# cesar-rocha/niwqg

Measured on NVIDIA B200. Metric: fp64 grid-point-steps/sec (coupled NIW-QG), higher is better.
Workload: dtype f64

## Files before the change

### niwqg_b200/csrc/kernels_fused.cuh

```cuda
#pragma once
#include "fft_split.cuh"
#include "kernels_family.cuh"

template <int N> struct FusedGeom {
    static constexpr int R = 16, M = N / R, Nh = N / 2;
    static constexpr int NB = Nh / 64;
    static constexpr int UNITS = (M / 2) * NB;
    static constexpr size_t XSMEM = (size_t)R * 256 * sizeof(cd);
};

struct FusedThread {
    int fam;
    int n;
    int side;
    int col;
    int ptid;
    int kzero;
};

template <int N>
__host__ __device__ __forceinline__ void fused_thread(int unit, int tid, const cd* __restrict__ twc, FusedThread& t) {
    using G = FusedGeom<N>;
    const int kk = unit / G::NB;
    int b = unit % G::NB, k;
    bool self;
    if (kk == 0) { self = true; if (b < G::NB / 2) k = 0; else { k = G::M / 2; b -= G::NB / 2; } }
    else { self = false; k = kk; }
    const int half = tid >> 7, wq = (tid >> 5) & 3, lane = tid & 31;
    t.side = lane >> 4;
    const int n0 = 64 * b + 16 * wq + (lane & 15);
    if (half == 0) { t.fam = k; t.n = n0; }
    else {
        t.fam = (G::M - k) % G::M;
        t.n = (n0 == 0) ? (self ? G::Nh / 2 : 0) : G::Nh - n0;
    }
    if (n0 != 0) t.ptid = tid ^ 128 ^ 16;
    else if (!self) t.ptid = tid ^ 128;
    else t.ptid = half ? (tid ^ 16) : tid;
    t.kzero = (t.fam == 0);
    t.col = t.n + t.side * G::Nh;
}
__host__ __device__ __forceinline__ int fused_qp(const FusedThread& t, int q) { return t.kzero ? ((16 - q) & 15) : 15 - q; }

__device__ __forceinline__ cd shfl16(cd v) {
    return make_double2(__shfl_xor_sync(0xffffffffu, v.x, 16), __shfl_xor_sync(0xffffffffu, v.y, 16));
}

template <int N>
__device__ __forceinline__ void fused_combine(const cd* __restrict__ T, const cd* __restrict__ twc, const FusedThread& t, cd (&u)[16]) {
    constexpr int M = N / 16;
    cd v[16];
    const cd wx = __ldg(&twc[t.n]), wy = __ldg(&twc[t.fam]);
#pragma unroll
    for (int r = 0; r < 16; ++r) v[r] = __ldg(&T[(size_t)(r * M + t.fam) * N + t.col]);
    if (t.side) {
#pragma unroll
        for (int r = 0; r < 16; ++r) v[r] = cmul(v[r], wx);
    }
#pragma unroll
    for (int r = 0; r < 16; ++r) {
        const cd o2 = shfl16(v[r]);
        v[r] = t.side ? csub(o2, v[r]) : cadd(v[r], o2);
    }
    fftc::apply_twiddles<16, 1>(v, wy);
    fftc::dft<16, 1>(v);
#pragma unroll
    for (int p = 0; p < 16; ++p) u[fftc::outidx<16>(p)] = v[p];
}

template <int N>
__device__ __forceinline__ void fused_produce(cd (&v)[16], const cd* __restrict__ twc, const FusedThread& t, int pro, double dk,
                                              cd* __restrict__ out) {
    constexpr int M = N / 16;
    const cd wx = __ldg(&twc[t.n]), wy = __ldg(&twc[t.fam]);
#define NIWQG_PRO_CASE(P)                                                                     \
    case P:                                                                                   \
        _Pragma("unroll") for (int r = 0; r < 16; ++r) v[r] = split_prologue<N, P>(dk, t.fam + M * r, t.col, v[r]); \
        break;
    switch (pro) {
        NIWQG_PRO_CASE(PRO_IK)
        NIWQG_PRO_CASE(PRO_IL)
        NIWQG_PRO_CASE(PRO_UV)
        default: break;
    }
#undef NIWQG_PRO_CASE
#pragma unroll
    for (int r = 0; r < 16; ++r) v[r].y = -v[r].y;
#pragma unroll
    for (int r = 0; r < 16; ++r) {
        const cd o2 = shfl16(v[r]);
        v[r] = t.side ? cmul(csub(o2, v[r]), wx) : cadd(v[r], o2);
    }
    fftc::dft<16, 1>(v);
    cd u[16];
#pragma unroll
    for (int p = 0; p < 16; ++p) u[fftc::outidx<16>(p)] = v[p];
    fftc::apply_twiddles<16, 1>(u, wy);
#pragma unroll
    for (int q = 0; q < 16; ++q) out[(size_t)(q * M + t.fam) * N + t.col] = u[q];
}

struct FStageArgs {
    StageArgs s;
    const cd* T;
    cd* out[3];
    int nout;
    const cd* twc;
    double dk;
};

struct EqIn { cd y0, cur, F0, Fab, y1, c0, c1, c2, c3; double fl; };

template <int ST, bool PHI>
__device__ __forceinline__ void eq_load(EqIn& in, const cd* __restrict__ y0, const cd* y, const cd* __restrict__ y1,
                                        const cd* __restrict__ F0, const cd* Fab, const TableSet& t,
                                        const double* __restrict__ filtr, size_t i) {
    in.y0 = __ldg(&y0[i]);
    if (PHI && ST >= 2) in.cur = (ST == 2) ? __ldg(&y1[i]) : y[i];
    if (ST >= 3) { in.F0 = __ldg(&F0[i]); in.Fab = (ST == 4) ? __ldg(&Fab[i]) : Fab[i]; }
    if (ST == 3) in.y1 = __ldg(&y1[i]);
    if (ST <= 3) { in.c0 = __ldg(&t.E2[i]); in.c1 = __ldg(&t.Q[i]); }
    else { in.c0 = __ldg(&t.E[i]); in.c1 = __ldg(&t.f0[i]); in.c2 = __ldg(&t.fab[i]); in.c3 = __ldg(&t.fc[i]); }
    in.fl = __ldg(&filtr[i]);
}
template <int ST> struct FusedDepth { static constexpr int Q = ST <= 2 ? 4 : 3, PHI = ST <= 2 ? 4 : (ST == 3 ? 3 : 2), INV = 6; };
template <int ST>
__device__ __forceinline__ cd eq_update(const EqIn& in, cd y0, cd Fn, cd& F0, cd& Fab) {
    cd r;
    if (ST == 1 || ST == 2) {
        r = cadd(cmul(in.c0, y0), cmul(Fn, in.c1));
        if (ST == 1) F0 = Fn; else Fab = Fn;
    } else if (ST == 3) {
        F0 = in.F0;
        const cd c = make_double2(2.0 * Fn.x - F0.x, 2.0 * Fn.y - F0.y);
        r = cadd(cmul(in.c0, in.y1), cmul(c, in.c1));
        Fab = cadd(in.Fab, Fn);
    } else {
        const cd ab2 = make_double2(2.0 * in.Fab.x, 2.0 * in.Fab.y);
        r = cadd(cadd(cadd(cmul(in.c0, y0), cmul(in.F0, in.c1)), cmul(ab2, in.c2)), cmul(Fn, in.c3));
    }
    return make_double2(r.x * in.fl, r.y * in.fl);
}

template <int N, int ST>
__global__ void __launch_bounds__(256, 2) k_fstage_q(FStageArgs a) {
    using G = FusedGeom<N>;
    constexpr int M = G::M;
    extern __shared__ __align__(16) unsigned char fused_smem[];
    cd* xs = reinterpret_cast<cd*>(fused_smem);
    const int tid = threadIdx.x;
    for (int unit = blockIdx.x; unit < G::UNITS; unit += gridDim.x) {
        FusedThread t;
        fused_thread<N>(unit, tid, a.twc, t);
        {
            cd u[16];
            fused_combine<N>(a.T, a.twc, t, u);
#pragma unroll
            for (int q = 0; q < 16; ++q) xs[q * 256 + tid] = u[q];
        }
        __syncthreads();
        const double k1 = a.dk * (double)sidx(t.col, N);
        const size_t i0 = (size_t)t.fam * N + t.col;
        constexpr int D = FusedDepth<ST>::Q;
        EqIn in[D];
        const int ub = unit % G::NB;
        const bool nyq = (ub == 0) || (unit < G::NB && ub == G::NB / 2);
        if (a.s.hsym && !t.kzero && !nyq) {
            const int colp = (N - t.col) & (N - 1);
#pragma unroll
            for (int p = 0; p < D - 1; ++p) eq_load<ST, false>(in[p], a.s.y0q, a.s.yq, a.s.y1q, a.s.F0q, a.s.Fabq, a.s.tq, a.s.filtr, i0 + (size_t)(2 * p) * M * N);
#pragma unroll
            for (int qq = 0; qq < 8; ++qq) {
                const int q = 2 * qq;
                const int ky = t.fam + M * q;
                const size_t i1 = i0 + (size_t)q * M * N;
                const size_t ip = (size_t)(N - ky) * N + colp;
                if (qq + D - 1 < 8) eq_load<ST, false>(in[(qq + D - 1) % D], a.s.y0q, a.s.yq, a.s.y1q, a.s.F0q, a.s.Fabq, a.s.tq, a.s.filtr, i1 + (size_t)(2 * (D - 1)) * M * N);
                const cd p1 = xs[q * 256 + tid], p2 = xs[(15 - q) * 256 + t.ptid];
                const double l1 = a.dk * (double)sidx(ky, N);
                const cd A = make_double2(0.5 * (p1.x + p2.x), 0.5 * (p1.y - p2.y));
                const cd B = make_double2(0.5 * (p1.y + p2.y), -0.5 * (p1.x - p2.x));
                const cd F1 = make_double2(k1 * A.y + l1 * B.y, -(k1 * A.x + l1 * B.x));
                const EqIn& e = in[qq % D];
                cd F0a, Faba;
                const cd n1 = eq_update<ST>(e, e.y0, F1, F0a, Faba);
                const cd n1c = make_double2(n1.x, -n1.y);
                a.s.yq[i1] = n1; a.s.yq[ip] = n1c;
                if (ST == 1) {
                    a.s.F0q[i1] = F0a; a.s.F0q[ip] = make_double2(F0a.x, -F0a.y);
                    if (a.s.y1q != a.s.yq) { a.s.y1q[i1] = n1; a.s.y1q[ip] = n1c; }
                }
                if (ST == 2 || ST == 3) { a.s.Fabq[i1] = Faba; a.s.Fabq[ip] = make_double2(Faba.x, -Faba.y); }
            }
            __syncthreads();
            continue;
        }
#pragma unroll
        for (int p = 0; p < D - 1; ++p) eq_load<ST, false>(in[p], a.s.y0q, a.s.yq, a.s.y1q, a.s.F0q, a.s.Fabq, a.s.tq, a.s.filtr, i0 + (size_t)p * M * N);
#pragma unroll
        for (int q = 0; q < 16; ++q) {
            const int ky = t.fam + M * q;
            const size_t i1 = i0 + (size_t)q * M * N;
            if (q + D - 1 < 16) eq_load<ST, false>(in[(q + D - 1) % D], a.s.y0q, a.s.yq, a.s.y1q, a.s.F0q, a.s.Fabq, a.s.tq, a.s.filtr, i1 + (size_t)(D - 1) * M * N);
            const cd p1 = xs[q * 256 + tid], p2 = xs[fused_qp(t, q) * 256 + t.ptid];
            const double l1 = a.dk * (double)sidx(ky, N);
            const cd A = make_double2(0.5 * (p1.x + p2.x), 0.5 * (p1.y - p2.y));
            const cd B = make_double2(0.5 * (p1.y + p2.y), -0.5 * (p1.x - p2.x));
            cd F1 = make_double2(k1 * A.y + l1 * B.y, -(k1 * A.x + l1 * B.x));
            if (ky == 0 && t.col == 0) F1 = make_double2(0.0, 0.0);
            const EqIn& e = in[q % D];
            cd F0a, Faba;
            const cd n1 = eq_update<ST>(e, e.y0, F1, F0a, Faba);
            a.s.yq[i1] = n1;
            if (ST == 1) { a.s.F0q[i1] = F0a; if (a.s.y1q != a.s.yq) a.s.y1q[i1] = n1; }
            if (ST == 2 || ST == 3) a.s.Fabq[i1] = Faba;
        }
        __syncthreads();
    }
}

template <int N, int ST>
__global__ void __launch_bounds__(256, 2) k_fstage_phi(FStageArgs a) {
    using G = FusedGeom<N>;
    constexpr int M = G::M;
    extern __shared__ __align__(16) unsigned char fused_smem[];
    cd* xs = reinterpret_cast<cd*>(fused_smem);
    const int tid = threadIdx.x;
    __shared__ double ssum[SE_COUNT][256];
#pragma unroll
    for (int k = 0; k < SE_COUNT; ++k) ssum[k][tid] = 0.0;
    const bool specb = (a.s.flags & MF_SPEC_BUDGET) != 0;
    for (int unit = blockIdx.x; unit < G::UNITS; unit += gridDim.x) {
        FusedThread t;
        fused_thread<N>(unit, tid, a.twc, t);
        {
            cd u[16];
            fused_combine<N>(a.T, a.twc, t, u);
#pragma unroll
            for (int q = 0; q < 16; ++q) xs[q * 256 + tid] = u[q];
        }
        __syncwarp();
        const double k1 = a.dk * (double)sidx(t.col, N);
        const size_t i0 = (size_t)t.fam * N + t.col;
        double s[SE_COUNT];
#pragma unroll
        for (int k = 0; k < SE_COUNT; ++k) s[k] = 0.0;
        constexpr int D = FusedDepth<ST>::PHI;
        EqIn in[D];
#pragma unroll
        for (int p = 0; p < D - 1; ++p) eq_load<ST, true>(in[p], a.s.y0p, a.s.yp, a.s.y1p, a.s.F0p, a.s.Fabp, a.s.tp, a.s.filtr, i0 + (size_t)p * M * N);
#pragma unroll
        for (int q = 0; q < 16; ++q) {
            const int ky = t.fam + M * q;
            const size_t i1 = i0 + (size_t)q * M * N;
            if (q + D - 1 < 16) eq_load<ST, true>(in[(q + D - 1) % D], a.s.y0p, a.s.yp, a.s.y1p, a.s.F0p, a.s.Fabp, a.s.tp, a.s.filtr, i1 + (size_t)(D - 1) * M * N);
            const EqIn& e = in[q % D];
            cd F1 = xs[q * 256 + tid];
            const cd cur1 = (ST == 1) ? e.y0 : e.cur;
            if (specb || (a.s.flags & MF_HAS_LAP2)) {
                const double l1 = a.dk * (double)sidx(ky, N);
                const double wv2 = k1 * k1 + l1 * l1, w4 = wv2 * wv2;
                const double m2 = cur1.x * cur1.x + cur1.y * cur1.y;
                s[SE_LAP2] += w4 * m2;
                s[SE_WV6PHI] += w4 * wv2 * m2;
                if (specb) {
                    const double zr = cur1.x * F1.x + cur1.y * F1.y, zi = cur1.y * F1.x - cur1.x * F1.y;
                    s[SE_T0R] += zr; s[SE_T0I] += zi;
                    s[SE_T1R] += wv2 * zr; s[SE_T1I] += wv2 * zi;
                    s[SE_T2R] += w4 * zr; s[SE_T2I] += w4 * zi;
                }
            }
            if ((a.s.flags & MF_FIX00) && ky == 0 && t.col == 0) { F1.x += a.s.sumsD[SD_J_R]; F1.y += a.s.sumsD[SD_J_I]; }
            cd F0a, Faba;
            const cd n1 = eq_update<ST>(e, e.y0, F1, F0a, Faba);
            a.s.yp[i1] = n1;
            if (ST == 1) { a.s.F0p[i1] = F0a; if (a.s.y1p != a.s.yp) a.s.y1p[i1] = n1; }
            if (ST == 2 || ST == 3) a.s.Fabp[i1] = Faba;
        }
#pragma unroll
        for (int k = 0; k < SE_COUNT; ++k) ssum[k][tid] += s[k];
        for (int o = 0; o < a.nout; ++o) {
            cd v[16];
#pragma unroll
            for (int r = 0; r < 16; ++r) v[r] = a.s.yp[i0 + (size_t)r * M * N];
            fused_produce<N>(v, a.twc, t, o == 0 ? PRO_NONE : o == 1 ? PRO_IK : PRO_IL, a.dk, a.out[o]);
        }
    }
    double s[SE_COUNT];
#pragma unroll
    for (int k = 0; k < SE_COUNT; ++k) s[k] = ssum[k][tid];
    block_reduce_store<SE_COUNT>(s, a.s.partials);
}

struct FInvertArgs {
    InvertArgs i;
    const cd* T;
    cd *out_uv, *out_qs;
    const cd* twc;
    double dk;
};

struct InvIn { cd q1, q2; double fl, flp; };

template <int N, bool HASW>
__global__ void __launch_bounds__(256, 2) k_finvert(FInvertArgs a) {
    using G = FusedGeom<N>;
    constexpr int M = G::M;
    extern __shared__ __align__(16) unsigned char fused_smem[];
    cd* xs = reinterpret_cast<cd*>(fused_smem);
    const int tid = threadIdx.x;
    __shared__ double ssum[SI_COUNT][256];
#pragma unroll
    for (int k = 0; k < SI_COUNT; ++k) ssum[k][tid] = 0.0;
    for (int unit = blockIdx.x; unit < G::UNITS; unit += gridDim.x) {
        FusedThread t;
        fused_thread<N>(unit, tid, a.twc, t);
        if (HASW) {
            cd u[16];
            fused_combine<N>(a.T, a.twc, t, u);
#pragma unroll
            for (int q = 0; q < 16; ++q) xs[q * 256 + tid] = u[q];
            __syncthreads();
        }
        cd u[16];
        double s[SI_COUNT] = {0.0, 0.0, 0.0};
        const double k1 = a.dk * (double)sidx(t.col, N);
        const int colp = (N - t.col) & (N - 1);
        const size_t i0 = (size_t)t.fam * N + t.col;
        auto load = [&](InvIn& in, int q) {
            const int ky = t.fam + M * q, kyp = (N - ky) & (N - 1);
            in.q1 = __ldg(&a.i.qh[i0 + (size_t)q * M * N]);
            in.q2 = __ldg(&a.i.qh[(size_t)kyp * N + colp]);
            if (HASW) {
                in.fl = __ldg(&a.i.filtr[i0 + (size_t)q * M * N]);
                in.flp = a.i.filtr_sym ? in.fl : __ldg(&a.i.filtr[(size_t)kyp * N + colp]);
            }
        };
        constexpr int D = FusedDepth<1>::INV;
        InvIn in[D];
#pragma unroll
        for (int p = 0; p < D - 1; ++p) load(in[p], p);
#pragma unroll
        for (int q = 0; q < 16; ++q) {
            const int ky = t.fam + M * q;
            const size_t i1 = i0 + (size_t)q * M * N;
            if (q + D - 1 < 16) load(in[(q + D - 1) % D], q + D - 1);
            const InvIn& e = in[q % D];
            const double l1 = a.dk * (double)sidx(ky, N);
            const double wv2 = __dadd_rn(__dmul_rn(k1, k1), __dmul_rn(l1, l1));
            const double wv2i = (wv2 != 0.0) ? 1.0 / wv2 : 0.0;
            const cd Hq = make_double2(0.5 * (e.q1.x + e.q2.x), 0.5 * (e.q1.y - e.q2.y));
            cd qw = make_double2(0.0, 0.0), qwr = qw;
            if (HASW) {
                const cd W1 = xs[q * 256 + tid], W2 = xs[fused_qp(t, q) * 256 + t.ptid];
                const cd A = make_double2(0.5 * (W1.x + W2.x), 0.5 * (W1.y - W2.y));
                cd Jc = make_double2(a.i.inv_jscale * 0.5 * (W1.y + W2.y), a.i.inv_jscale * -0.5 * (W1.x - W2.x));
                if (ky == 0 && t.col == 0) Jc = make_double2(0.0, 0.0);
                const double bx = 0.5 * (0.5 * (-wv2 * A.x) + Jc.x) / a.i.f, by = 0.5 * (0.5 * (-wv2 * A.y) + Jc.y) / a.i.f;
                const double fs = 0.5 * (e.fl + e.flp);
                qw.x = bx * fs; qw.y = by * fs;
                qwr.x = bx * e.fl; qwr.y = by * e.fl;
            }
            const cd ph1 = make_double2(wv2i * qw.x - wv2i * Hq.x, wv2i * qw.y - wv2i * Hq.y);
            {
                const double r = Hq.x * ph1.x + Hq.y * ph1.y;
                s[SI_QLAP2PSI] += wv2 * wv2 * r;
                s[SI_PLAPQ] += -wv2 * r;
                s[SI_PQ] += r;
            }
            a.i.ph[i1] = ph1;
            if (a.i.qwh) a.i.qwh[i1] = qwr;
            u[q] = make_double2(Hq.x - qw.y, Hq.y + qw.x);
        }
        if (HASW) __syncthreads();
#pragma unroll
        for (int k = 0; k < SI_COUNT; ++k) ssum[k][tid] += s[k];
        fused_produce<N>(u, a.twc, t, PRO_NONE, a.dk, a.out_qs);
#pragma unroll
        for (int r = 0; r < 16; ++r) u[r] = a.i.ph[i0 + (size_t)r * M * N];
        fused_produce<N>(u, a.twc, t, PRO_UV, a.dk, a.out_uv);
    }
    double s[SI_COUNT];
#pragma unroll
    for (int k = 0; k < SI_COUNT; ++k) s[k] = ssum[k][tid];
    block_reduce_store<SI_COUNT>(s, a.i.partials);
}

template <int N>
static cudaError_t fused_set_attrs() {
    static bool attr_set[64] = {};
    int dev = 0;
    cudaGetDevice(&dev);
    if (dev < 64 && attr_set[dev]) return cudaSuccess;
    const int sm = (int)FusedGeom<N>::XSMEM;
    cudaError_t e;
#define NIWQG_ATTR(K) if ((e = cudaFuncSetAttribute(K, cudaFuncAttributeMaxDynamicSharedMemorySize, sm)) != cudaSuccess) return e;
    NIWQG_ATTR((k_fstage_q<N, 1>)) NIWQG_ATTR((k_fstage_q<N, 2>)) NIWQG_ATTR((k_fstage_q<N, 3>)) NIWQG_ATTR((k_fstage_q<N, 4>))
    NIWQG_ATTR((k_fstage_phi<N, 1>)) NIWQG_ATTR((k_fstage_phi<N, 2>)) NIWQG_ATTR((k_fstage_phi<N, 3>)) NIWQG_ATTR((k_fstage_phi<N, 4>))
    NIWQG_ATTR((k_finvert<N, true>))
#undef NIWQG_ATTR
    if (dev < 64) attr_set[dev] = true;
    return cudaSuccess;
}

template <int N>
static cudaError_t launch_fstage(const FStageArgs& a, bool phi, int grid, cudaStream_t st) {
    cudaError_t e = fused_set_attrs<N>();
    if (e != cudaSuccess) return e;
    const size_t sm = FusedGeom<N>::XSMEM;
    if (phi) {
        switch (a.s.stage) {
            case 1: k_fstage_phi<N, 1><<<grid, 256, sm, st>>>(a); break;
            case 2: k_fstage_phi<N, 2><<<grid, 256, sm, st>>>(a); break;
            case 3: k_fstage_phi<N, 3><<<grid, 256, sm, st>>>(a); break;
            default: k_fstage_phi<N, 4><<<grid, 256, sm, st>>>(a); break;
        }
    } else {
        switch (a.s.stage) {
            case 1: k_fstage_q<N, 1><<<grid, 256, sm, st>>>(a); break;
            case 2: k_fstage_q<N, 2><<<grid, 256, sm, st>>>(a); break;
            case 3: k_fstage_q<N, 3><<<grid, 256, sm, st>>>(a); break;
            default: k_fstage_q<N, 4><<<grid, 256, sm, st>>>(a); break;
        }
    }
    return cudaGetLastError();
}

template <int N>
static cudaError_t launch_finvert(const FInvertArgs& a, bool has_w, int grid, cudaStream_t st) {
    cudaError_t e = fused_set_attrs<N>();
    if (e != cudaSuccess) return e;
    if (has_w) k_finvert<N, true><<<grid, 256, FusedGeom<N>::XSMEM, st>>>(a);
    else k_finvert<N, false><<<grid, 256, 0, st>>>(a);
    return cudaGetLastError();
}
```

Measured before the change: 1.272 billion.

## Prefetch next unit's FFT input tile via TMA bulk copies with mbarriers

Replaces the per-thread strided global loads of the 16 FFT input rows in the fused stage/invert kernels with async bulk (TMA) copies into shared memory. The copies are tracked by per-half mbarriers and issued for the next unit while the current one is computed. Shared memory is re-laid out so the combine output and the staged tile share slots. This is meant to hide global load latency and coalesce accesses. In exchange it adds more dynamic shared memory per block, which may reduce occupancy, plus extra barrier and proxy-fence complexity.

```diff
diff --git a/niwqg_b200/csrc/kernels_fused.cuh b/niwqg_b200/csrc/kernels_fused.cuh
--- a/niwqg_b200/csrc/kernels_fused.cuh
+++ b/niwqg_b200/csrc/kernels_fused.cuh
@@ -7,6 +7,8 @@
     static constexpr int NB = Nh / 64;
     static constexpr int UNITS = (M / 2) * NB;
     static constexpr size_t XSMEM = (size_t)R * 256 * sizeof(cd);
+    static constexpr size_t TSMEM = (size_t)R * 128 * sizeof(cd);
+    static constexpr int TS = R * 256;
 };
 
 struct FusedThread {
@@ -16,17 +18,33 @@
     int col;
     int ptid;
     int kzero;
+    int half;
+    int xs, pxs;
+    int ts;
 };
+
+__host__ __device__ __forceinline__ int fused_slot(int tid) {
+    const int half = tid >> 7, side = (tid >> 4) & 1, c = ((tid >> 5) & 3) * 16 + (tid & 15);
+    return half * 2048 + side * 64 + (half ? 63 - c : c);
+}
+
+template <int N>
+__host__ __device__ __forceinline__ void fused_unit(int unit, int& k, int& b, bool& self) {
+    using G = FusedGeom<N>;
+    const int kk = unit / G::NB;
+    b = unit % G::NB;
+    if (kk == 0) { self = true; if (b < G::NB / 2) k = 0; else { k = G::M / 2; b -= G::NB / 2; } }
+    else { self = false; k = kk; }
+}
 
 template <int N>
 __host__ __device__ __forceinline__ void fused_thread(int unit, int tid, const cd* __restrict__ twc, FusedThread& t) {
     using G = FusedGeom<N>;
-    const int kk = unit / G::NB;
-    int b = unit % G::NB, k;
+    int b, k;
     bool self;
-    if (kk == 0) { self = true; if (b < G::NB / 2) k = 0; else { k = G::M / 2; b -= G::NB / 2; } }
-    else { self = false; k = kk; }
+    fused_unit<N>(unit, k, b, self);
     const int half = tid >> 7, wq = (tid >> 5) & 3, lane = tid & 31;
+    t.half = half;
     t.side = lane >> 4;
     const int n0 = 64 * b + 16 * wq + (lane & 15);
     if (half == 0) { t.fam = k; t.n = n0; }
@@ -39,20 +57,73 @@
     else t.ptid = half ? (tid ^ 16) : tid;
     t.kzero = (t.fam == 0);
     t.col = t.n + t.side * G::Nh;
+    t.xs = fused_slot(tid);
+    t.pxs = fused_slot(t.ptid);
+    t.ts = half ? t.xs : G::TS + t.xs;
 }
 __host__ __device__ __forceinline__ int fused_qp(const FusedThread& t, int q) { return t.kzero ? ((16 - q) & 15) : 15 - q; }
+
+template <int N>
+__host__ __device__ __forceinline__ void fused_tile_seg(int unit, int half, int r, int side, size_t& src, int& len, size_t& src1) {
+    using G = FusedGeom<N>;
+    int k, b;
+    bool self;
+    fused_unit<N>(unit, k, b, self);
+    const int fam = half ? (G::M - k) % G::M : k;
+    const size_t row = (size_t)(r * G::M + fam) * N + (size_t)side * G::Nh;
+    src1 = 0;
+    len = 64;
+    if (!half) src = row + 64 * b;
+    else if (b > 0) src = row + G::Nh - 64 * b - 63;
+    else { src = row + G::Nh - 63; len = 63; src1 = row + (self ? G::Nh / 2 : 0); }
+}
+
+template <int N>
+__device__ __forceinline__ void fused_tile_load(const cd* T, int unit, int half, cd* smem, unsigned long long* bars) {
+    const int lane = (int)threadIdx.x - 128 * half;
+    if (lane < 0 || lane >= 32 || unit >= FusedGeom<N>::UNITS) return;
+    const int r = lane >> 1, side = lane & 1;
+    size_t src, src1;
+    int len;
+    fused_tile_seg<N>(unit, half, r, side, src, len, src1);
+    const unsigned bar = smem_u32(&bars[half]);
+    if (lane == 0) mbar_expect_tx(bar, 32 * 64 * sizeof(cd));
+    __syncwarp();
+    const unsigned d = smem_u32(smem + (half ? 2048 : FusedGeom<N>::TS) + r * 128 + side * 64);
+    bulk_load(d, T + src, len * sizeof(cd), bar);
+    if (len < 64) bulk_load(d + 63 * sizeof(cd), T + src1, sizeof(cd), bar);
+}
+
+__device__ __forceinline__ void fused_half_sync(int half) { asm volatile("bar.sync %0, 128;" ::"r"(1 + half) : "memory"); }
+
+template <int N>
+__device__ __forceinline__ void fused_tile_start(const cd* T, cd* smem, unsigned long long* bars) {
+    if (threadIdx.x == 0) { mbar_init(smem_u32(&bars[0]), 1); mbar_init(smem_u32(&bars[1]), 1); }
+    __syncthreads();
+    fused_tile_load<N>(T, blockIdx.x, 0, smem, bars);
+    fused_tile_load<N>(T, blockIdx.x, 1, smem, bars);
+}
+
+template <int N, bool WHOLE>
+__device__ __forceinline__ void fused_release_xs(const cd* T, int next, cd* smem, unsigned long long* bars) {
+    asm volatile("fence.proxy.async.shared::cta;" ::: "memory");
+    if (WHOLE) __syncthreads();
+    else fused_half_sync(1);
+    fused_tile_load<N>(T, next, 1, smem, bars);
+}
 
 __device__ __forceinline__ cd shfl16(cd v) {
     return make_double2(__shfl_xor_sync(0xffffffffu, v.x, 16), __shfl_xor_sync(0xffffffffu, v.y, 16));
 }
 
 template <int N>
-__device__ __forceinline__ void fused_combine(const cd* __restrict__ T, const cd* __restrict__ twc, const FusedThread& t, cd (&u)[16]) {
-    constexpr int M = N / 16;
+__device__ __forceinline__ void fused_combine(cd* smem, unsigned long long* bars, int unit, const cd* __restrict__ twc,
+                                              const FusedThread& t) {
     cd v[16];
     const cd wx = __ldg(&twc[t.n]), wy = __ldg(&twc[t.fam]);
-#pragma unroll
-    for (int r = 0; r < 16; ++r) v[r] = __ldg(&T[(size_t)(r * M + t.fam) * N + t.col]);
+    mbar_wait(smem_u32(&bars[t.half]), ((unit - blockIdx.x) / gridDim.x) & 1);
+#pragma unroll
+    for (int r = 0; r < 16; ++r) v[r] = smem[t.ts + 128 * r];
     if (t.side) {
 #pragma unroll
         for (int r = 0; r < 16; ++r) v[r] = cmul(v[r], wx);
@@ -65,7 +136,7 @@
     fftc::apply_twiddles<16, 1>(v, wy);
     fftc::dft<16, 1>(v);
 #pragma unroll
-    for (int p = 0; p < 16; ++p) u[fftc::outidx<16>(p)] = v[p];
+    for (int p = 0; p < 16; ++p) smem[t.xs + 128 * fftc::outidx<16>(p)] = v[p];
 }
 
 template <int N>
@@ -147,18 +218,16 @@
     using G = FusedGeom<N>;
     constexpr int M = G::M;
     extern __shared__ __align__(16) unsigned char fused_smem[];
+    __shared__ unsigned long long bars[2];
     cd* xs = reinterpret_cast<cd*>(fused_smem);
     const int tid = threadIdx.x;
+    fused_tile_start<N>(a.T, xs, bars);
     for (int unit = blockIdx.x; unit < G::UNITS; unit += gridDim.x) {
         FusedThread t;
         fused_thread<N>(unit, tid, a.twc, t);
-        {
-            cd u[16];
-            fused_combine<N>(a.T, a.twc, t, u);
-#pragma unroll
-            for (int q = 0; q < 16; ++q) xs[q * 256 + tid] = u[q];
-        }
+        fused_combine<N>(xs, bars, unit, a.twc, t);
         __syncthreads();
+        fused_tile_load<N>(a.T, unit + gridDim.x, 0, xs, bars);
         const double k1 = a.dk * (double)sidx(t.col, N);
         const size_t i0 = (size_t)t.fam * N + t.col;
         constexpr int D = FusedDepth<ST>::Q;
@@ -176,7 +245,7 @@
                 const size_t i1 = i0 + (size_t)q * M * N;
                 const size_t ip = (size_t)(N - ky) * N + colp;
                 if (qq + D - 1 < 8) eq_load<ST, false>(in[(qq + D - 1) % D], a.s.y0q, a.s.yq, a.s.y1q, a.s.F0q, a.s.Fabq, a.s.tq, a.s.filtr, i1 + (size_t)(2 * (D - 1)) * M * N);
-                const cd p1 = xs[q * 256 + tid], p2 = xs[(15 - q) * 256 + t.ptid];
+                const cd p1 = xs[t.xs + 128 * q], p2 = xs[t.pxs + 128 * (15 - q)];
                 const double l1 = a.dk * (double)sidx(ky, N);
                 const cd A = make_double2(0.5 * (p1.x + p2.x), 0.5 * (p1.y - p2.y));
                 const cd B = make_double2(0.5 * (p1.y + p2.y), -0.5 * (p1.x - p2.x));
@@ -192,7 +261,7 @@
                 }
                 if (ST == 2 || ST == 3) { a.s.Fabq[i1] = Faba; a.s.Fabq[ip] = make_double2(Faba.x, -Faba.y); }
             }
-            __syncthreads();
+            fused_release_xs<N, true>(a.T, unit + gridDim.x, xs, bars);
             continue;
         }
 #pragma unroll
@@ -202,7 +271,7 @@
             const int ky = t.fam + M * q;
             const size_t i1 = i0 + (size_t)q * M * N;
             if (q + D - 1 < 16) eq_load<ST, false>(in[(q + D - 1) % D], a.s.y0q, a.s.yq, a.s.y1q, a.s.F0q, a.s.Fabq, a.s.tq, a.s.filtr, i1 + (size_t)(D - 1) * M * N);
-            const cd p1 = xs[q * 256 + tid], p2 = xs[fused_qp(t, q) * 256 + t.ptid];
+            const cd p1 = xs[t.xs + 128 * q], p2 = xs[t.pxs + 128 * fused_qp(t, q)];
             const double l1 = a.dk * (double)sidx(ky, N);
             const cd A = make_double2(0.5 * (p1.x + p2.x), 0.5 * (p1.y - p2.y));
             const cd B = make_double2(0.5 * (p1.y + p2.y), -0.5 * (p1.x - p2.x));
@@ -215,7 +284,7 @@
             if (ST == 1) { a.s.F0q[i1] = F0a; if (a.s.y1q != a.s.yq) a.s.y1q[i1] = n1; }
             if (ST == 2 || ST == 3) a.s.Fabq[i1] = Faba;
         }
-        __syncthreads();
+        fused_release_xs<N, true>(a.T, unit + gridDim.x, xs, bars);
     }
 }
 
@@ -230,16 +299,17 @@
 #pragma unroll
     for (int k = 0; k < SE_COUNT; ++k) ssum[k][tid] = 0.0;
     const bool specb = (a.s.flags & MF_SPEC_BUDGET) != 0;
+    __shared__ unsigned long long bars[2];
+    fused_tile_start<N>(a.T, xs, bars);
     for (int unit = blockIdx.x; unit < G::UNITS; unit += gridDim.x) {
         FusedThread t;
         fused_thread<N>(unit, tid, a.twc, t);
-        {
-            cd u[16];
-            fused_combine<N>(a.T, a.twc, t, u);
-#pragma unroll
-            for (int q = 0; q < 16; ++q) xs[q * 256 + tid] = u[q];
-        }
-        __syncwarp();
+        fused_combine<N>(xs, bars, unit, a.twc, t);
+        if (t.half) __syncwarp();
+        else {
+            fused_half_sync(0);
+            fused_tile_load<N>(a.T, unit + gridDim.x, 0, xs, bars);
+        }
         const double k1 = a.dk * (double)sidx(t.col, N);
         const size_t i0 = (size_t)t.fam * N + t.col;
         double s[SE_COUNT];
@@ -255,7 +325,7 @@
             const size_t i1 = i0 + (size_t)q * M * N;
             if (q + D - 1 < 16) eq_load<ST, true>(in[(q + D - 1) % D], a.s.y0p, a.s.yp, a.s.y1p, a.s.F0p, a.s.Fabp, a.s.tp, a.s.filtr, i1 + (size_t)(D - 1) * M * N);
             const EqIn& e = in[q % D];
-            cd F1 = xs[q * 256 + tid];
+            cd F1 = xs[t.xs + 128 * q];
             const cd cur1 = (ST == 1) ? e.y0 : e.cur;
             if (specb || (a.s.flags & MF_HAS_LAP2)) {
                 const double l1 = a.dk * (double)sidx(ky, N);
@@ -279,6 +349,7 @@
         }
 #pragma unroll
         for (int k = 0; k < SE_COUNT; ++k) ssum[k][tid] += s[k];
+        if (t.half) fused_release_xs<N, false>(a.T, unit + gridDim.x, xs, bars);
         for (int o = 0; o < a.nout; ++o) {
             cd v[16];
 #pragma unroll
@@ -312,15 +383,15 @@
     __shared__ double ssum[SI_COUNT][256];
 #pragma unroll
     for (int k = 0; k < SI_COUNT; ++k) ssum[k][tid] = 0.0;
+    __shared__ unsigned long long bars[2];
+    if (HASW) fused_tile_start<N>(a.T, xs, bars);
     for (int unit = blockIdx.x; unit < G::UNITS; unit += gridDim.x) {
         FusedThread t;
         fused_thread<N>(unit, tid, a.twc, t);
         if (HASW) {
-            cd u[16];
-            fused_combine<N>(a.T, a.twc, t, u);
-#pragma unroll
-            for (int q = 0; q < 16; ++q) xs[q * 256 + tid] = u[q];
+            fused_combine<N>(xs, bars, unit, a.twc, t);
             __syncthreads();
+            fused_tile_load<N>(a.T, unit + gridDim.x, 0, xs, bars);
         }
         cd u[16];
         double s[SI_COUNT] = {0.0, 0.0, 0.0};
@@ -352,7 +423,7 @@
             const cd Hq = make_double2(0.5 * (e.q1.x + e.q2.x), 0.5 * (e.q1.y - e.q2.y));
             cd qw = make_double2(0.0, 0.0), qwr = qw;
             if (HASW) {
-                const cd W1 = xs[q * 256 + tid], W2 = xs[fused_qp(t, q) * 256 + t.ptid];
+                const cd W1 = xs[t.xs + 128 * q], W2 = xs[t.pxs + 128 * fused_qp(t, q)];
                 const cd A = make_double2(0.5 * (W1.x + W2.x), 0.5 * (W1.y - W2.y));
                 cd Jc = make_double2(a.i.inv_jscale * 0.5 * (W1.y + W2.y), a.i.inv_jscale * -0.5 * (W1.x - W2.x));
                 if (ky == 0 && t.col == 0) Jc = make_double2(0.0, 0.0);
@@ -372,7 +443,7 @@
             if (a.i.qwh) a.i.qwh[i1] = qwr;
             u[q] = make_double2(Hq.x - qw.y, Hq.y + qw.x);
         }
-        if (HASW) __syncthreads();
+        if (HASW) fused_release_xs<N, true>(a.T, unit + gridDim.x, xs, bars);
 #pragma unroll
         for (int k = 0; k < SI_COUNT; ++k) ssum[k][tid] += s[k];
         fused_produce<N>(u, a.twc, t, PRO_NONE, a.dk, a.out_qs);
@@ -392,7 +463,7 @@
     int dev = 0;
     cudaGetDevice(&dev);
     if (dev < 64 && attr_set[dev]) return cudaSuccess;
-    const int sm = (int)FusedGeom<N>::XSMEM;
+    const int sm = (int)(FusedGeom<N>::XSMEM + FusedGeom<N>::TSMEM);
     cudaError_t e;
 #define NIWQG_ATTR(K) if ((e = cudaFuncSetAttribute(K, cudaFuncAttributeMaxDynamicSharedMemorySize, sm)) != cudaSuccess) return e;
     NIWQG_ATTR((k_fstage_q<N, 1>)) NIWQG_ATTR((k_fstage_q<N, 2>)) NIWQG_ATTR((k_fstage_q<N, 3>)) NIWQG_ATTR((k_fstage_q<N, 4>))
@@ -407,7 +478,7 @@
 static cudaError_t launch_fstage(const FStageArgs& a, bool phi, int grid, cudaStream_t st) {
     cudaError_t e = fused_set_attrs<N>();
     if (e != cudaSuccess) return e;
-    const size_t sm = FusedGeom<N>::XSMEM;
+    const size_t sm = FusedGeom<N>::XSMEM + FusedGeom<N>::TSMEM;
     if (phi) {
         switch (a.s.stage) {
             case 1: k_fstage_phi<N, 1><<<grid, 256, sm, st>>>(a); break;
@@ -430,7 +501,7 @@
 static cudaError_t launch_finvert(const FInvertArgs& a, bool has_w, int grid, cudaStream_t st) {
     cudaError_t e = fused_set_attrs<N>();
     if (e != cudaSuccess) return e;
-    if (has_w) k_finvert<N, true><<<grid, 256, FusedGeom<N>::XSMEM, st>>>(a);
+    if (has_w) k_finvert<N, true><<<grid, 256, FusedGeom<N>::XSMEM + FusedGeom<N>::TSMEM, st>>>(a);
     else k_finvert<N, false><<<grid, 256, 0, st>>>(a);
     return cudaGetLastError();
 }
```

Result: slower. 1.211 billion (median of 6 runs) (-4.8%).
